# smn-ailab/PyCMF

Measured on AMD Instinct MI355X. Metric: factor-update iterations/s (mu solver: one full update_step per iteration), higher is better.
Workload: dtype f32

## Files before the change

### include/cmfhip.h

```cpp
#ifndef CMFHIP_H
#define CMFHIP_H

#include <stdint.h>

#ifdef __cplusplus
extern "C" {
#endif

typedef struct cmf_ctx cmf_ctx;

enum {
    CMF_OK = 0,
    CMF_EINVAL = 1,
    CMF_EHIP = 2,
    CMF_ENOMEM = 3,
    CMF_ENODEV = 4,
    CMF_EUNSUPPORTED = 5,
    CMF_ERCCL = 6
};

enum { CMF_U = 0, CMF_V = 1, CMF_Z = 2 };
enum { CMF_LINK_LINEAR = 0, CMF_LINK_LOGIT = 1 };
enum { CMF_UPD_U = 1, CMF_UPD_V = 2, CMF_UPD_Z = 4 };
enum { CMF_NN_U = 1, CMF_NN_V = 2, CMF_NN_Z = 4 };
// ... 68 lines not shown
int cmf_weighted_residual_sq(cmf_ctx *ctx, double *ex, double *ey);
int cmf_mu_weighted_layout(cmf_ctx *ctx, int64_t *out4);
int cmf_fill_weight_synthetic(cmf_ctx *ctx, int which, uint64_t seed, double density);
int cmf_get_weight_block_f32(cmf_ctx *ctx, int which, int64_t row0, int64_t nrows, int64_t col0, int64_t ncols, float *host_dst);

int cmf_hals_step(cmf_ctx *ctx, double l1, double l2, int update_mask);
int cmf_hals_sweep(cmf_ctx *ctx, int which, const double *N, const double *G, double l1, double l2);

int cmf_als_step(cmf_ctx *ctx, double l2, int nn_mask, int update_mask);
int cmf_als_normal(cmf_ctx *ctx, int which, int64_t row0, int64_t nrows, double l2, float *host_H, float *host_g);
int cmf_als_layout(cmf_ctx *ctx, int64_t *out4);
int cmf_als_nnls_step(cmf_ctx *ctx, double l2, int nn_mask, int update_mask, int sweeps);
int cmf_als_nnls_rows(cmf_ctx *ctx, int64_t nrows, const float *host_H, const float *host_g, float *host_f, int sweeps);
int cmf_als_cg_step(cmf_ctx *ctx, double l2, int nn_mask, int update_mask, int cg_steps, int nn_sweeps);
int cmf_als_cg_rows(cmf_ctx *ctx, int which, int64_t row0, int64_t nrows, double l2, int cg_steps, float *host_f);
int cmf_als_cg_last(cmf_ctx *ctx, int64_t *out2);

int cmf_set_background_weight(cmf_ctx *ctx, int which, double c0);
int cmf_get_background_weight(cmf_ctx *ctx, int which, double *c0);
int cmf_als_residual_sq(cmf_ctx *ctx, double *ex, double *ey);

int cmf_set_biases(cmf_ctx *ctx, int which, int enable, double mu, double lb);
int cmf_get_biases(cmf_ctx *ctx, int which, double *mu, double *lb, int *enabled);
int cmf_set_bias_f64(cmf_ctx *ctx, int which, int axis, const double *v);
int cmf_get_bias_f64(cmf_ctx *ctx, int which, int axis, double *v);
int cmf_als_bias_step(cmf_ctx *ctx, double l2, int nn_mask, int update_mask, int cg_steps, int nn_sweeps);
int cmf_als_bias_rows(cmf_ctx *ctx, int which, int axis, float *host_out);
int cmf_als_bias_targets(cmf_ctx *ctx, int which, int image, int64_t nnz, float *host_bt, float *host_bp);
int cmf_predict_pairs(cmf_ctx *ctx, int which, int link, int64_t n, const int64_t *rows, const int64_t *cols, float *out);

int cmf_v_buf_elems(cmf_ctx *ctx, int64_t *n);
int cmf_mu_v_partials(cmf_ctx *ctx, float *dev_buf);
int cmf_data_pass_launches(cmf_ctx *ctx, int64_t *out5);
int cmf_mu_route_launches(cmf_ctx *ctx, int64_t *out8);
int cmf_mu_v_partials_rows(cmf_ctx *ctx, float *dev_buf, int64_t row0, int64_t nrows, int with_gram);
int cmf_mu_v_apply(cmf_ctx *ctx, const float *dev_buf, double l1, double l2);
int cmf_mu_uz_update(cmf_ctx *ctx, double l1, double l2, int update_mask);
int cmf_mu_blocked_layout(cmf_ctx *ctx, int world, int64_t *block_rows, int64_t *pbuf_elems);
int cmf_mu_v_partials_split(cmf_ctx *ctx, float *dev_P, float *dev_G);
int cmf_mu_v_apply_rows(cmf_ctx *ctx, const float *dev_P_rows, const float *dev_G, int64_t row0, int64_t nrows, double l1, double l2);
int cmf_mu_gram_v_rows(cmf_ctx *ctx, int64_t row0, int64_t nrows, float *dev_G2);
int cmf_mu_uz_update_gram(cmf_ctx *ctx, const float *dev_G2, double l1, double l2, int update_mask);

int cmf_newton_step(cmf_ctx *ctx, double alpha, double l1, double l2,
                    int x_link, int y_link, int nn_mask, int update_mask,
                    double hessian_pertubation, double sg_ratio,
                    const int32_t *u_idx, const int32_t *z_idx,
                    const int32_t *vx_idx, const int32_t *vy_idx);

int cmf_newton_step_device_sampled(cmf_ctx *ctx, double alpha, double l1, double l2,
                                   int x_link, int y_link, int nn_mask, int update_mask,
                                   double hessian_pertubation, double sg_ratio, uint64_t seed);

int cmf_sample_lists(cmf_ctx *ctx, int sweep, uint64_t seed, double sg_ratio, int64_t row0, int64_t nrows, int32_t *host_out);

int cmf_newton_uz_update(cmf_ctx *ctx, double alpha, double l1, double l2,
                         int nn_mask, int update_mask, double hessian_pertubation);
int cmf_newton_v_partials(cmf_ctx *ctx, double alpha, float *dev_buf);
int cmf_newton_v_apply(cmf_ctx *ctx, const float *dev_buf, double l1, double l2,
                       int nn_mask, double hessian_pertubation);

int cmf_newton_v_gram(cmf_ctx *ctx, double alpha, double *dev_gbuf);
int cmf_newton_v_products(cmf_ctx *ctx, double alpha, double l2, double hessian_pertubation,
                          const double *dev_gbuf, float *dev_pbuf);
int cmf_newton_v_finish(cmf_ctx *ctx, float *dev_pbuf, double l1, int nn_mask);

// ... 90 lines not shown
```

### pycmf_amd/_lib.py

```python
import ctypes as C
import os

import numpy as np

_HERE = os.path.dirname(os.path.abspath(__file__))
LIB_PATH = os.path.join(_HERE, "libcmfhip.so")

CMF_U, CMF_V, CMF_Z = 0, 1, 2
CMF_UPD_U, CMF_UPD_V, CMF_UPD_Z = 1, 2, 4
CMF_NN_U, CMF_NN_V, CMF_NN_Z = 1, 2, 4
LINKS = {"linear": 0, "logit": 1}
UPD_U, UPD_V, UPD_Z = 1, 2, 4
K_GEMM_NN, K_GEMM_TN, K_GEMM_NT, K_ELEMWISE, K_EIGEN = 0, 1, 2, 3, 4
KERNEL_CLASSES = {"gemm_nn": 0, "gemm_tn": 1, "gemm_nt": 2, "elementwise": 3, "eigen": 4, "gemm_small": 5, "spmm": 6, "rowhess": 7, "gemm_pair": 8, "topk": 9, "klmu": 10}
LATER_KERNEL_CLASSES = {"hals": 11}

_ERR = {1: ValueError, 2: RuntimeError, 3: MemoryError, 4: RuntimeError, 5: NotImplementedError}

_i64, _i32, _dbl, _vp = C.c_int64, C.c_int, C.c_double, C.c_void_p
_pd = C.POINTER(C.c_double)
_pf = C.POINTER(C.c_float)
_pi32 = C.POINTER(C.c_int32)
_pi64 = C.POINTER(C.c_int64)

# ... 34 lines not shown
    "cmf_mu_beta_layout": [_vp, _pi64],
    "cmf_set_weight_f64": [_vp, _i32, _pd, _i64, _i64],
    "cmf_set_weight_f32": [_vp, _i32, _pf, _i64, _i64],
    "cmf_set_weighted_csr": [_vp, _i32, _pi64, _pi32, _pd, _pd],
    "cmf_clear_weight": [_vp, _i32],
    "cmf_mu_weighted_step": [_vp, _dbl, _dbl, _i32],
    "cmf_weighted_residual_sq": [_vp, _pd, _pd],
    "cmf_mu_weighted_layout": [_vp, _pi64],
    "cmf_fill_weight_synthetic": [_vp, _i32, C.c_uint64, _dbl],
    "cmf_get_weight_block_f32": [_vp, _i32, _i64, _i64, _i64, _i64, _pf],
    "cmf_hals_step": [_vp, _dbl, _dbl, _i32],
    "cmf_hals_sweep": [_vp, _i32, _pd, _pd, _dbl, _dbl],
    "cmf_als_step": [_vp, _dbl, _i32, _i32],
    "cmf_als_normal": [_vp, _i32, _i64, _i64, _dbl, _pf, _pf],
    "cmf_als_layout": [_vp, _pi64],
    "cmf_als_nnls_step": [_vp, _dbl, _i32, _i32, _i32],
    "cmf_als_nnls_rows": [_vp, _i64, _pf, _pf, _pf, _i32],
    "cmf_als_cg_step": [_vp, _dbl, _i32, _i32, _i32, _i32],
    "cmf_als_cg_rows": [_vp, _i32, _i64, _i64, _dbl, _i32, _pf],
    "cmf_als_cg_last": [_vp, _pi64],
    "cmf_set_background_weight": [_vp, _i32, _dbl],
    "cmf_get_background_weight": [_vp, _i32, _pd],
    "cmf_als_residual_sq": [_vp, _pd, _pd],
    "cmf_set_biases": [_vp, _i32, _i32, _dbl, _dbl],
    "cmf_get_biases": [_vp, _i32, _pd, _pd, C.POINTER(C.c_int)],
    "cmf_set_bias_f64": [_vp, _i32, _i32, _pd],
    "cmf_get_bias_f64": [_vp, _i32, _i32, _pd],
    "cmf_als_bias_step": [_vp, _dbl, _i32, _i32, _i32, _i32],
    "cmf_als_bias_rows": [_vp, _i32, _i32, _pf],
    "cmf_als_bias_targets": [_vp, _i32, _i32, _i64, _pf, _pf],
    "cmf_predict_pairs": [_vp, _i32, _i32, _i64, _pi64, _pi64, _pf],
    "cmf_v_buf_elems": [_vp, _pi64],
    "cmf_data_pass_launches": [_vp, _pi64],
    "cmf_mu_route_launches": [_vp, _pi64],
    "cmf_mu_v_partials": [_vp, _vp],
    "cmf_mu_v_apply": [_vp, _vp, _dbl, _dbl],
    "cmf_mu_v_partials_rows": [_vp, _vp, _i64, _i64, _i32],
    "cmf_mu_uz_update": [_vp, _dbl, _dbl, _i32],
    "cmf_mu_blocked_layout": [_vp, _i32, _pi64, _pi64],
    "cmf_mu_v_partials_split": [_vp, _vp, _vp],
    "cmf_mu_v_apply_rows": [_vp, _vp, _vp, _i64, _i64, _dbl, _dbl],
    "cmf_mu_gram_v_rows": [_vp, _i64, _i64, _vp],
    "cmf_mu_uz_update_gram": [_vp, _vp, _dbl, _dbl, _i32],
    "cmf_newton_step": [_vp, _dbl, _dbl, _dbl, _i32, _i32, _i32, _i32, _dbl, _dbl,
                        _pi32, _pi32, _pi32, _pi32],
    "cmf_newton_step_device_sampled": [_vp, _dbl, _dbl, _dbl, _i32, _i32, _i32, _i32, _dbl, _dbl, C.c_uint64],
    "cmf_newton_uz_update": [_vp, _dbl, _dbl, _dbl, _i32, _i32, _dbl],
    "cmf_newton_v_partials": [_vp, _dbl, _vp],
    "cmf_newton_v_apply": [_vp, _vp, _dbl, _dbl, _i32, _dbl],
    "cmf_newton_v_gram": [_vp, _dbl, _vp],
    "cmf_newton_v_products": [_vp, _dbl, _dbl, _dbl, _vp, _vp],
    "cmf_newton_v_finish": [_vp, _vp, _dbl, _i32],
    "cmf_residual_sq": [_vp, _i32, _i32, _pd, _pd],
    "cmf_data_sq": [_vp, _pd, _pd],
    "cmf_topk": [_vp, _i32, _i32, _i32, _pi64, _i64, _i32, _pi64, _pi32, _pi32, _pf],
    "cmf_topk_queries": [_vp, _pd, _i64, _i64, _i64, _i32, _i32, _i32, _pi64, _pi32, _pi32, _pf],
    "cmf_topk_layout": [_vp, _i64, _i32, _i32, _i64, _i32, _pi64],
    "cmf_rank": [_vp, _i32, _i32, _pi64, _i64, _pi64, _pi32, _pi64, _pi32, _pi32, _pf, _pi32],
    "cmf_rank_queries": [_vp, _pd, _i64, _i64, _i64, _i32, _pi64, _pi32, _pi64, _pi32, _pi32, _pf, _pi32],
    "cmf_rank_layout": [_vp, _i64, _i32, _i64, _i64, _i32, _pi64],
    "cmf_safe_invert_batch": [_vp, _pd, _pd, _i32, _i32, _dbl],
    "cmf_safe_invert_f64": [_vp, _pd, _pd, _i32, _dbl],
    "cmf_safe_solve_batch": [_vp, _pd, _pd, _pd, _pd, _i32, _i32, _dbl, _i32],
    "cmf_debug_clock": [_vp, _pd, _pd],
    "cmf_kernel_timing": [_vp, _i32],
    "cmf_kernel_time": [_vp, _i32, _pd, _pi64, _pd],
# ... 485 lines not shown
    def als_bias_targets(self, which, image, nnz):
        nnz = int(nnz)
        if nnz < 0:
            raise ValueError("als_bias_targets: nnz must be the number of stored entries, got %d" % nnz)
        bt, bp = np.zeros(nnz, dtype=np.float32), np.zeros(nnz, dtype=np.float32)
        check(self._lib.cmf_als_bias_targets(self._h, which, image, nnz, bt.ctypes.data_as(_pf), bp.ctypes.data_as(_pf)))
        return bt, bp

    def predict_pairs(self, which, rows, cols, link="linear"):
        rows = np.ascontiguousarray(rows, dtype=np.int64).ravel()
        cols = np.ascontiguousarray(cols, dtype=np.int64).ravel()
        if rows.shape != cols.shape:
            raise ValueError("predict_pairs: rows and cols must have one length, got %d and %d" % (rows.size, cols.size))
        out = np.zeros(rows.size, dtype=np.float32)
        check(self._lib.cmf_predict_pairs(self._h, which, LINKS[link] if isinstance(link, str) else int(link), rows.size,
                                          rows.ctypes.data_as(_pi64), cols.ctypes.data_as(_pi64), out.ctypes.data_as(_pf)))
        return out

    def mu_step_error(self, l1, l2, mask=7):
        ex2, ey2 = C.c_double(0), C.c_double(0)
        check(self._lib.cmf_mu_step_error(self._h, l1, l2, mask, C.byref(ex2), C.byref(ey2)))
        return ex2.value, ey2.value

    def v_buf_elems(self):
        n = C.c_int64(0)
        check(self._lib.cmf_v_buf_elems(self._h, C.byref(n)))
        return n.value

    def data_pass_launches(self):
        out = np.zeros(5, dtype=np.int64)
        check(self._lib.cmf_data_pass_launches(self._h, out.ctypes.data_as(_pi64)))
        return tuple(int(v) for v in out)

    MU_ROUTE_FORMS = ("epi_mu", "factor_update", "factor_update2", "pair", "gram32", "sum_slabs", "mu_apply", "narrow_copy")

    def mu_route_launches(self):
        out = np.zeros(8, dtype=np.int64)
        check(self._lib.cmf_mu_route_launches(self._h, out.ctypes.data_as(_pi64)))
        return dict(zip(self.MU_ROUTE_FORMS, (int(v) for v in out)))

    def mu_v_partials(self, dev_ptr):
        check(self._lib.cmf_mu_v_partials(self._h, _vp(dev_ptr)))

    def mu_v_partials_rows(self, dev_ptr, row0, nrows, with_gram):
        check(self._lib.cmf_mu_v_partials_rows(self._h, _vp(dev_ptr), row0, nrows, 1 if with_gram else 0))

    def mu_v_apply(self, dev_ptr, l1, l2):
        check(self._lib.cmf_mu_v_apply(self._h, _vp(dev_ptr), l1, l2))

    def mu_uz_update(self, l1, l2, mask=7):
        check(self._lib.cmf_mu_uz_update(self._h, l1, l2, mask))

    def mu_blocked_layout(self, world):
        b, n = C.c_int64(0), C.c_int64(0)
        check(self._lib.cmf_mu_blocked_layout(self._h, int(world), C.byref(b), C.byref(n)))
        return b.value, n.value

    def mu_v_partials_split(self, dev_p, dev_g):
        check(self._lib.cmf_mu_v_partials_split(self._h, _vp(dev_p), _vp(dev_g)))

    def mu_v_apply_rows(self, dev_p_rows, dev_g, row0, nrows, l1, l2):
        check(self._lib.cmf_mu_v_apply_rows(self._h, _vp(dev_p_rows), _vp(dev_g), row0, nrows, l1, l2))

    def mu_gram_v_rows(self, row0, nrows, dev_g2):
        check(self._lib.cmf_mu_gram_v_rows(self._h, row0, nrows, _vp(dev_g2)))

# ... 327 lines not shown
```

### pycmf_amd/csrc/cmf_api.hip

```cpp
#include "../../include/cmfhip.h"
#include "cmf_kernels.hip.h"
#include "cmf_gemm_wg256.hip.h"
#include "cmf_gemm_pair.hip.h"
#include "cmf_eigen.hip.h"
#include "cmf_chol_mfma.hip.h"
#include "cmf_sparse.hip.h"
#include "cmf_rowhess.hip.h"
#include "cmf_bf16x6.hip.h"
#include "cmf_rowhess6.hip.h"
#include "cmf_shared64.hip.h"
#include "cmf_refine64.hip.h"
#include "cmf_eigclamp.hip.h"
#include "cmf_rank1clamp.hip.h"

#include <hip/hip_runtime.h>

#include <algorithm>
#include <chrono>
#include <cmath>
#include <cstdarg>
#include <cstdio>
#include <cstdlib>
#include <cstring>
#include <mutex>
// ... 74 lines not shown
struct StepGraph {
    hipGraphExec_t exec = nullptr;
    double key[8] = {0};
    int warm = 0;
    bool failed = false;
};

struct EvPair {
    hipEvent_t a, b;
    int cls;
    double flops;
};

struct CmfComm;
struct cmf_ctx {
    int device = 0;
    CmfComm *comm = nullptr;
    hipStream_t stream = nullptr;
    bool own_stream = false;
    int num_cu = 256;

    int64_t m = 0, d = 0, p = 0;
    int k = 0;
    int64_t mp = 0, dp = 0, pp = 0;
    int kp = 0;
    bool have_problem = false;
    unsigned long long *dbg_stamps = nullptr;
    bool diag_ok = false;
    int opt_graph = -1;
    StepGraph mu_graph, newton_graph;
    int opt_split = -1;
    int opt_data_pass_wg = 15;
    int64_t data_pass_launches[5] = {0, 0, 0, 0, 0};
    int64_t mu_route_launches[8] = {0, 0, 0, 0, 0, 0, 0, 0};
    int opt_pair = 1;
    int opt_arith_min_tiles = 8;
    int opt_arith = 0;
    int opt_ns = 1;
    bool hess_psd = true;
    int opt_pipe_nt = 4;
    int opt_topk_split = 0;
    int opt_kl_split = 0;
    DevBuf kl_slab, kl_small, kl_part;
    int opt_beta_route = 0;
    DevBuf beta_slab, beta_small, beta_part;
    int opt_wmu_split = 0;
    int wm_kind[2] = {0, 0};
    float *wm_w[2] = {nullptr, nullptr}, *wm_p[2] = {nullptr, nullptr};
    WCsrDev wm_sp[2][2];
    DevBuf wm_slab, wm_small, wm_part;
    DevBuf hals_ws;
    int opt_als_piece = 0;
    DevBuf als_h, als_part, als_g, als_sol, als_desc;
    DevBuf als_nnls_ws;
    int opt_als_cg_lds = -1;
    DevBuf als_cg_ws;
    int opt_als_cg_piece = 0;
    DevBuf als_cg_long;
    int64_t als_cg_last[2] = {0, 0};
    double wm_bg[2] = {0.0, 0.0};
    DevBuf als_bg_s, als_bg64;
    AlsBias als_bias[2];
    int opt_als_bias_piece = 0;
    DevBuf als_bias_part, als_bias_ws;
    int opt_choldiag = 0;
    int opt_chol = 1;
// ... 250 lines not shown
struct GemmPlan {
    int bn;
    int ntiles_n;
    int64_t tiles_m;
    int nsplit;
    int64_t klen;
};

static GemmPlan plan_gemm(const cmf_ctx *c, int64_t mout, int64_t n, int64_t kred, bool allow_split) {
    GemmPlan pl;
    pl.bn = n >= 256 ? 256 : (int)n;
    pl.ntiles_n = (int)(n / pl.bn);
    pl.tiles_m = (mout + 255) / 256;
    const int64_t tiles = pl.tiles_m * pl.ntiles_n;
    int64_t s = 1;
    if (allow_split && c->opt_split > 0) {
        s = std::min<int64_t>(c->opt_split, std::max<int64_t>(1, kred / 32));
    } else if (allow_split && tiles < (int64_t)(c->num_cu * 3) / 4) {
        s = ((int64_t)c->num_cu + tiles / 2) / tiles;
        const int64_t maxs = std::max<int64_t>(1, kred / 128);
        s = std::max<int64_t>(1, std::min(s, maxs));
    }
    pl.klen = rup((kred + s - 1) / s, 32);
    pl.nsplit = (int)((kred + pl.klen - 1) / pl.klen);
    return pl;
}

template <int MODE, int ROLE>
static int launch_gemm(cmf_ctx *c, const GemmArgs &a, const GemmPlan &pl) {
    static_assert(MODE != MODE_NT, "NT passes: gemm_nt");
    dim3 grid((unsigned)pl.tiles_m, (unsigned)pl.ntiles_n, (unsigned)pl.nsplit);
    if (ROLE == 0 && pl.bn == 256 && (c->opt_data_pass_wg & (MODE == MODE_TN ? 1 : 2)) && a.epi == EPI_NONE && a.Mout % 256 == 0) {
        if ((c->opt_data_pass_wg & (MODE == MODE_TN ? 4 : 8)) && a.lda < ((int64_t)1 << 21) && a.ldb < ((int64_t)1 << 21)) {
            using Cfg = Wg256Cfg<MODE, true>;
            if constexpr (Cfg::LDS_BYTES != 0) CHK(allow_big_lds(c, reinterpret_cast<const void *>(&gemm_wg256_kernel<MODE, true>), (int)Cfg::LDS_BYTES));
            hipLaunchKernelGGL((gemm_wg256_kernel<MODE, true>), grid, dim3(Cfg::NT), Cfg::LDS_BYTES, c->stream, a);
            ++c->data_pass_launches[MODE == MODE_TN ? 3 : 4];
        } else {
            using Cfg = Wg256Cfg<MODE, false>;
            CHK(allow_big_lds(c, reinterpret_cast<const void *>(&gemm_wg256_kernel<MODE, false>), (int)Cfg::LDS_BYTES));
            hipLaunchKernelGGL((gemm_wg256_kernel<MODE, false>), grid, dim3(Cfg::NT), Cfg::LDS_BYTES, c->stream, a);
            ++c->data_pass_launches[MODE == MODE_TN ? 1 : 2];
        }
        HIPCHK(hipGetLastError());
        return CMF_OK;
    }
    if (ROLE == 0 && pl.bn == 256) ++c->data_pass_launches[0];
    dim3 block(512);
#define CMF_LAUNCH(BN_)                                                                          \
    do {                                                                                         \
        using Cfg = GemmCfg<MODE, BN_>;                                                          \
        CHK(allow_big_lds(c, reinterpret_cast<const void *>(&gemm_kernel<MODE, BN_, ROLE, 4>), (int)Cfg::LDS_BYTES)); \
        hipLaunchKernelGGL((gemm_kernel<MODE, BN_, ROLE, 4>), grid, block, Cfg::LDS_BYTES, c->stream, a); \
    } while (0)
    switch (pl.bn) {
    case 256: CMF_LAUNCH(256); break;
    case 128: CMF_LAUNCH(128); break;
    case 64: CMF_LAUNCH(64); break;
    case 32: CMF_LAUNCH(32); break;
    default: return fail(CMF_EINVAL, "unsupported tile width %d", pl.bn);
    }
#undef CMF_LAUNCH
    HIPCHK(hipGetLastError());
    return CMF_OK;
}

static int sum_slabs(cmf_ctx *c, float *dst, const float *src, int64_t n, int nslab, int64_t stride,
                     bool accumulate) {
    Timed tm(c, CMF_K_ELEMWISE);
    const int64_t n4 = n / 4;
    const int blocks = (int)std::min<int64_t>((n4 + 255) / 256, 2048);
    hipLaunchKernelGGL(sum_slabs_kernel, dim3(blocks), dim3(256), 0, c->stream, dst, src, n4, nslab, stride,
                       accumulate ? 1 : 0);
    ++c->mu_route_launches[5];
    HIPCHK(hipGetLastError());
    return CMF_OK;
}

static int mu_apply(cmf_ctx *c, float *F, const float *num, const float *den, int64_t n, double l1, double l2);

struct SlabRef {
    const float *base = nullptr;
    int nslab = 0;
    int64_t stride = 0;
    int64_t quota = 0, unit0 = 0;
    int ksteps = 0;
};

struct Epilogue {
    int kind = 0;
    const float *F = nullptr, *P = nullptr;
    const SlabRef *Pslabs = nullptr, *Pslabs2 = nullptr;
    float *out = nullptr;
    double a = 0.0, b = 0.0, c = 0.0;
    int64_t rows = 0;
    int kvalid = 0, nn = 0;
};

static int gemm(cmf_ctx *c, int mode, const float *A, int64_t lda, const float *B, int64_t ldb, float *out,
                int64_t mout, int64_t n, int64_t kred, bool accumulate = false, const Epilogue *mu = nullptr, SlabRef *defer = nullptr) {
    const bool data_pass = (lda != c->kp);
    DevBuf &slabbuf = c->slab_sel ? c->slabs_b : c->slabs;
    if (kred % 32 || n % 32) return fail(CMF_EINVAL, "gemm: unpadded extent (k=%lld n=%lld)", (long long)kred, (long long)n);
    GemmPlan pl = plan_gemm(c, mout, n, kred, mu == nullptr);
    if (mu && c->opt_narrow_update && pl.ntiles_n == 1) {
        while (pl.bn > 64 && pl.tiles_m * (n / pl.bn) * 2 <= (int64_t)c->num_cu) pl.bn /= 2;
// ... 301 lines not shown
extern "C" int cmf_comm_destroy(cmf_ctx *c);
extern "C" int cmf_ctx_destroy(cmf_ctx *c) {
    if (!c) return CMF_OK;
    DeviceGuard dg(c->device);
    (void)cmf_comm_destroy(c);
    release_problem(c);
    for (void *p : c->scratch) (void)hipFree(p);
    c->scratch.clear();
    (void)hipFree(c->dscalar);
    for (auto &e : c->pending) { (void)hipEventDestroy(e.a); (void)hipEventDestroy(e.b); }
    for (auto e : c->evpool) (void)hipEventDestroy(e);
    for (auto e : c->markers) (void)hipEventDestroy(e);
    for (int b = 0; b < 2; ++b) {
        pin_give(c->pin[b]);
        if (c->pin_ev[b]) (void)hipEventDestroy(c->pin_ev[b]);
    }
    if (c->own_stream) (void)hipStreamDestroy(c->stream);
    delete c;
    return CMF_OK;
}

extern "C" int cmf_set_option(cmf_ctx *c, const char *name, int64_t value) {
    if (!c || !name) return fail(CMF_EINVAL, "null argument");
    invalidate_graphs(c);
    if (!strcmp(name, "graph")) {
        c->opt_graph = value < 0 ? -1 : (value != 0);
        return CMF_OK;
    }
    if (!strcmp(name, "gemm_pipe_nt")) {
        c->opt_pipe_nt = (int)value;
    } else if (!strcmp(name, "gemm_split")) {
        c->opt_split = (int)value;
    } else if (!strcmp(name, "data_pass_wg")) {
        if (value < 0 || value > 15)
            return fail(CMF_EINVAL, "data_pass_wg: bit 0 the TN data passes, bit 1 the NN data passes, bit 2 / bit 3 their factor from a register ring (0..15)");
        c->opt_data_pass_wg = (int)value;
    } else if (!strcmp(name, "small_gram_shares")) {
        c->opt_gram32_shares = (int)std::max<int64_t>(1, std::min<int64_t>(value, 1024));
    } else if (!strcmp(name, "small_gram")) {
        c->opt_gram32 = value != 0;
    } else if (!strcmp(name, "chol_mfma")) {
        c->opt_chol_mfma = value != 0;
    } else if (!strcmp(name, "narrow_update")) {
        c->opt_narrow_update = value != 0;
    } else if (!strcmp(name, "pair_passes")) {
        c->opt_pair = (int)value;
    } else if (!strcmp(name, "z_logit_hessian_l2")) {
        c->opt_zlogit_l2 = value != 0;
    } else if (!strcmp(name, "row_diag")) {
#ifndef CMF_DIAG_BUILD
        if (value != 0) return fail(CMF_EINVAL, "row_diag is a timing-only diagnostic (wrong results) that the default build does not carry: "
                                                "build with `python -m pycmf_amd.build --diag` and set CMF_DIAG=1");
#endif
        if (value != 0 && !c->diag_ok) return fail(CMF_EINVAL, "row_diag is a timing-only diagnostic (wrong results): set CMF_DIAG=1 in the environment to allow it");
        c->opt_rowdiag = (int)value;
    } else if (!strcmp(name, "row_stagger")) {
        c->opt_rowstagger = value != 0;
    } else if (!strcmp(name, "row_symmetric")) {
        c->opt_rowsym = (int)value;
    } else if (!strcmp(name, "row_kernel")) {
        c->opt_rowkernel = value != 0;
    } else if (!strcmp(name, "direct_newton_step")) {
        c->opt_direct_step = value != 0;
    } else if (!strcmp(name, "row_certificates")) {
        c->opt_rowcert = value != 0;
    } else if (!strcmp(name, "row_classes")) {
        if (value < -1 || value > 6) return fail(CMF_EINVAL, "row_classes: -1 (automatic), 0 (off) or 2..6 rows per group");
        c->opt_rowclasses = (int)value;
    } else if (!strcmp(name, "row_chunk")) {
// ... 461 lines not shown
    (void)hipFree(dev_ptr);
    return CMF_OK;
}

extern "C" int cmf_export_factor_rows(cmf_ctx *c, int which, float *dev_dst) {
    NEED_PROBLEM(c);
    if (which < 0 || which > 2 || !dev_dst) return fail(CMF_EINVAL, "bad factor argument");
    DeviceGuard dg(c->device);
    HIPCHK(hipMemcpyAsync(dev_dst, c->F[which], (size_t)c->frows[which] * c->kp * sizeof(float), hipMemcpyDeviceToDevice, c->stream));
    return CMF_OK;
}

extern "C" int cmf_import_factor_rows(cmf_ctx *c, int which, const float *dev_src) {
    NEED_PROBLEM(c);
    if (which < 0 || which > 2 || !dev_src) return fail(CMF_EINVAL, "bad factor argument");
    DeviceGuard dg(c->device);
    HIPCHK(hipMemcpyAsync(c->F[which], dev_src, (size_t)c->frows[which] * c->kp * sizeof(float), hipMemcpyDeviceToDevice, c->stream));
    return CMF_OK;
}

extern "C" int cmf_v_buf_elems(cmf_ctx *c, int64_t *n) {
    NEED_PROBLEM(c);
    if (!n) return fail(CMF_EINVAL, "null argument");
    *n = c->dp * c->kp + (int64_t)c->kp * c->kp;
    return CMF_OK;
}

extern "C" int cmf_data_pass_launches(cmf_ctx *c, int64_t *out5) {
    if (!c || !out5) return fail(CMF_EINVAL, "cmf_data_pass_launches: null context or output");
    for (int f = 0; f < 5; ++f) out5[f] = c->data_pass_launches[f];
    return CMF_OK;
}

extern "C" int cmf_mu_route_launches(cmf_ctx *c, int64_t *out8) {
    if (!c || !out8) return fail(CMF_EINVAL, "cmf_mu_route_launches: null context or output");
    for (int f = 0; f < 8; ++f) out8[f] = c->mu_route_launches[f];
    return CMF_OK;
}

extern "C" int cmf_mu_v_partials(cmf_ctx *c, float *buf) {
    NEED_PROBLEM(c);
    if (!buf) return fail(CMF_EINVAL, "null buffer");
    if (!have_data(c, 0) || !have_data(c, 1)) return fail(CMF_EINVAL, "X and Y must be set before a V update");
    DeviceGuard dg(c->device);
    float *P = buf, *Gs = buf + c->dp * c->kp;
    CHK(data_times(c, 0, true, c->F[CMF_U], P));
    CHK(data_times(c, 1, false, c->F[CMF_Z], P, true));
    CHK(gram32(c, c->F[CMF_U], c->mp + c->pp, Gs));
    return CMF_OK;
}

extern "C" int cmf_mu_v_partials_rows(cmf_ctx *c, float *buf, int64_t row0, int64_t nrows, int with_gram) {
    NEED_PROBLEM(c);
    if (!buf) return fail(CMF_EINVAL, "null buffer");
    if (!c->X || !c->Y) return fail(CMF_EUNSUPPORTED, "cmf_mu_v_partials_rows needs dense images of X and Y");
    if (c->opt_arith != 0) return fail(CMF_EUNSUPPORTED, "cmf_mu_v_partials_rows: fp32 MFMA arithmetic only");
    if (row0 < 0 || nrows <= 0 || row0 % 256 || nrows % 256 || row0 + nrows > c->dp) return fail(CMF_EINVAL, "row block must be 256-aligned inside [0, d_pad)");
    DeviceGuard dg(c->device);
    float *P = buf + row0 * c->kp;
    CHK(gemm(c, MODE_TN, c->X + row0, c->dp, c->F[CMF_U], c->kp, P, nrows, c->kp, c->mp));
    CHK(gemm(c, MODE_NN, c->Y + row0 * c->pp, c->pp, c->F[CMF_Z], c->kp, P, nrows, c->kp, c->pp, true));
    if (with_gram)
        CHK(gram32(c, c->F[CMF_U], c->mp + c->pp, buf + c->dp * c->kp));
    return CMF_OK;
}

// ... 443 lines not shown
```

### pycmf_amd/csrc/cmf_gemm_wg256.hip.h

```cpp
#pragma once
#include "cmf_kernels.hip.h"

namespace cmfk {

template <int MODE, bool FREG>
struct Wg256Cfg {
    static_assert(MODE == MODE_NN || MODE == MODE_TN, "data passes: NN and TN");
    static constexpr int BM = 256, BN = 256, BK = 32, PADK = BK + 4, NT = 256;
    static constexpr int A_ELEMS = (MODE == MODE_NN) ? BM * PADK : 0;
    static constexpr int B_ELEMS = FREG ? 0 : BK * BN;
    static constexpr int STAGE = A_ELEMS + B_ELEMS;
    static constexpr int LD = BK * BN / 4 / NT;
    static constexpr size_t LDS_BYTES = 2 * STAGE * sizeof(float);
};

template <int MODE, bool FREG>
__global__ __launch_bounds__(256) void gemm_wg256_kernel(GemmArgs g) {
    using C = Wg256Cfg<MODE, FREG>;
    constexpr bool NN = (MODE == MODE_NN);
    constexpr bool LDS = C::LDS_BYTES != 0;
    constexpr int NGRP = C::BK / 2;
    constexpr int XREG_MI = 5, FREG_MI = 10;
    extern __shared__ __attribute__((aligned(16))) float smem[];

    const int t = threadIdx.x;
    const int lane = t & 63, wid = t >> 6;
    const int l31 = lane & 31, lh = lane >> 5;
    const int wrow0 = 128 * (wid >> 1), wcol0 = 128 * (wid & 1);

    const int64_t row0 = (int64_t)blockIdx.x * C::BM;
    const int64_t n0 = (int64_t)blockIdx.y * C::BN;
    const int64_t kbeg = (int64_t)blockIdx.z * g.klen;
    int64_t kend = kbeg + g.klen;
    if (kend > g.Kred) kend = g.Kred;
    const int nkt = (int)((kend - kbeg) / C::BK);
    const int64_t klast = kend - C::BK;

    f32x16 acc[4][4];
#pragma unroll
    for (int i = 0; i < 4; ++i)
#pragma unroll
        for (int j = 0; j < 4; ++j)
#pragma unroll
            for (int r = 0; r < 16; ++r) acc[i][j][r] = 0.0f;

    const int64_t wg_linear = ((int64_t)blockIdx.z * gridDim.y + blockIdx.y) * gridDim.x + blockIdx.x;
    if (g.dbg && t == 0) {
        g.dbg[4 * wg_linear + 0] = __builtin_amdgcn_s_memtime();
        g.dbg[4 * wg_linear + 1] = __builtin_amdgcn_s_memrealtime();
    }

    f32x4 rb[FREG ? 1 : C::LD], ra[NN ? C::LD : 1];
// ... 45 lines not shown
#pragma unroll
                for (int s = 0; s < NGRP; ++s) gload_x(kbeg, s);
        } else if constexpr (NN) {
#pragma unroll
            for (int p = 0; p < C::LD; ++p) gload_au(kbeg, p);
            __builtin_amdgcn_sched_barrier(0);
#pragma unroll
            for (int p = 0; p < C::LD; ++p) lstore_a(smem, p);
            __builtin_amdgcn_sched_barrier(0);
#pragma unroll
            for (int p = 0; p < C::LD; ++p) {
                gload_au(k1, p);
                __builtin_amdgcn_sched_barrier(0);
                if (p == FREG_MI / 2 - 1) {
                    gload_f(kbeg, 0);
                    __builtin_amdgcn_sched_barrier(0);
                }
            }
#pragma unroll
            for (int s = 1; s < NGRP - 1; ++s) {
                gload_f(kbeg, s);
                __builtin_amdgcn_sched_barrier(0);
            }
        } else {
#pragma unroll
            for (int s = 0; s < NGRP - 1; ++s) {
                gload_xu(kbeg, s);
                __builtin_amdgcn_sched_barrier(0);
                gload_f(kbeg, s);
                __builtin_amdgcn_sched_barrier(0);
            }
        }
        if constexpr (LDS) __syncthreads();
        for (int kt = 0; kt < nkt; ++kt) {
            const float *As = smem + (kt & 1) * C::STAGE, *Bs = As + C::A_ELEMS;
            float *nAs = smem + ((kt + 1) & 1) * C::STAGE, *nBs = nAs + C::A_ELEMS;
            int64_t kn1 = kbeg + (int64_t)(kt + 1) * C::BK, kn2 = kn1 + C::BK;
            kn1 = kn1 < klast ? kn1 : klast;
            kn2 = kn2 < klast ? kn2 : klast;
            f32x4 a[NN ? 2 : 1][4], b[2];
            auto ldb_frag = [&](int sidx) {
                const int kk = NN ? 8 * (sidx >> 2) + 4 * lh + (sidx & 3) : 2 * sidx + lh;
                b[sidx & 1] = *reinterpret_cast<const f32x4 *>(Bs + kk * C::BN + wcol0 + 4 * l31);
            };
            auto lda_frag = [&](int q) {
#pragma unroll
                for (int i = 0; i < 4; ++i)
                    a[q & 1][i] = *reinterpret_cast<const f32x4 *>(As + (wrow0 + 32 * i + l31) * C::PADK + 4 * (2 * q + lh));
            };
            if constexpr (NN) lda_frag(0);
            if constexpr (!FREG) ldb_frag(0);
#pragma unroll
            for (int sidx = 0; sidx < NGRP; ++sidx) {
                const int q = sidx >> 2, e = sidx & 3;
                if (sidx + 1 < NGRP) {
                    if constexpr (!FREG) ldb_frag(sidx + 1);
                    if constexpr (NN)
                        if (e == 0 && q + 1 < NGRP / 4) lda_frag(q + 1);
                }
                __builtin_amdgcn_sched_barrier(0);
#pragma unroll
                for (int mi = 0; mi < 16; ++mi) {
                    const int i = mi >> 2, j = mi & 3;
                    const float av = NN ? a[q & 1][i][e] : xr[sidx][i];
                    const float bv = FREG ? br[sidx][j] : b[sidx & 1][j];
                    acc[i][j] = __builtin_amdgcn_mfma_f32_32x32x2f32(av, bv, acc[i][j], 0, 0, 0);
                    if constexpr (NN && FREG) {
                        if (sidx == 0 && (mi & 1)) lstore_a(nAs, mi >> 1);
                        if (sidx == 1 && (mi & 1)) gload_au(kn2, mi >> 1);
                    } else if constexpr (NN) {
                        const int p = mi >> 1;
                        if (sidx == 0) {
                            if (mi & 1) lstore_b(nBs, p);
                            else lstore_a(nAs, p);
                        } else if (sidx == 1) {
                            if (mi & 1) gload_b(kn2, p);
                            else gload_a(kn2, p);
                        }
                    } else if constexpr (!FREG) {
                        if (sidx == 0 && mi < C::LD) lstore_b(nBs, mi);
                        if (sidx == 0 && mi >= C::LD) gload_b(kn2, mi - C::LD);
                    }
                    if constexpr (FREG) {
                        const int rs = (sidx + NGRP - 1) % NGRP;
                        const int64_t kr = sidx == 0 ? kbeg + (int64_t)kt * C::BK : kn1;
                        if (!NN && mi == XREG_MI) gload_xu(kr, rs);
                        if (mi == FREG_MI) gload_f(kr, rs);
                    }
                    __builtin_amdgcn_sched_barrier(0);
                }
                if constexpr (!NN && !FREG) {
                    gload_x(kn1, sidx);
                    __builtin_amdgcn_sched_barrier(0);
                }
            }
            if constexpr (LDS) __syncthreads();
        }
    }

    if (g.dbg && t == 0) {
        g.dbg[4 * wg_linear + 2] = __builtin_amdgcn_s_memtime();
        g.dbg[4 * wg_linear + 3] = __builtin_amdgcn_s_memrealtime();
    }
    const bool in_red = g.red_out != nullptr;
    float *Cl = (in_red ? g.red_out : g.C + (int64_t)blockIdx.z * g.slab_stride) +
                (row0 + wrow0 + (NN ? 4 : 16) * lh) * g.ldc + n0 + wcol0 + 4 * l31;
    const int ldc = (int)g.ldc;
    auto rowoff = [&](int i, int r) -> int {
        const int rr = (r & 3) + 8 * (r >> 2);
        return (NN ? 32 * i + rr : 4 * rr + i) * ldc;
    };
    if (in_red && g.red_acc) {
#pragma unroll
        for (int i = 0; i < 4; ++i) {
#pragma unroll
            for (int j = 0; j < 4; ++j) asm volatile("" : "+a"(acc[i][j]));
            f32x4 old[16];
#pragma unroll
            for (int r = 0; r < 16; ++r) old[r] = *reinterpret_cast<const f32x4 *>(Cl + rowoff(i, r));
#pragma unroll
            for (int r = 0; r < 16; ++r) {
                f32x4 v = {acc[i][0][r], acc[i][1][r], acc[i][2][r], acc[i][3][r]};
                v += old[r];
                *reinterpret_cast<f32x4 *>(Cl + rowoff(i, r)) = v;
            }
            __builtin_amdgcn_sched_barrier(0);
        }
    } else {
#pragma unroll
// ... 15 lines not shown
```

### pycmf_amd/csrc/cmf_kernels.hip.h

```cpp
#pragma once
#include <hip/hip_runtime.h>
#include <stdint.h>

namespace cmfk {

typedef float f32x16 __attribute__((ext_vector_type(16)));
typedef float f32x4 __attribute__((ext_vector_type(4)));
typedef float f32x2 __attribute__((ext_vector_type(2)));

enum { MODE_NN = 0, MODE_TN = 1, MODE_NT = 2 };

struct GemmArgs {
    const float *A;
    int64_t lda;
    const float *B;
    int64_t ldb;
    float *C;
    int64_t ldc;
    int64_t slab_stride;
    int64_t Mout;
    int64_t Kred;
    int64_t klen;
    const float *T;
    int64_t ldt;
// ... 731 lines not shown
    for (int idx = blockIdx.x * 256 + threadIdx.x; idx < kp * kp; idx += gridDim.x * 256) {
        const int r = idx / kp, c = idx % kp;
        const int rr = r < c ? r : c, cc = r < c ? c : r;
        const int ti = rr / ts, tj = cc / ts;
        int ir = rr % ts, ic = cc % ts;
        if (ti == tj) { ir = r % ts; ic = c % ts; }
        const int tile = ti * T - ti * (ti - 1) / 2 + (tj - ti);
        const float *p = slab + (int64_t)tile * ts * ts + ir * ts + ic;
        const int64_t st = (int64_t)ntile * ts * ts;
        float s = 0.f;
        int q = 0;
        for (; q + 8 <= nsplit; q += 8) {
            float v[8];
#pragma unroll
            for (int u = 0; u < 8; ++u) v[u] = p[(q + u) * st];
#pragma unroll
            for (int u = 0; u < 8; ++u) s += v[u];
        }
        for (; q < nsplit; ++q) s += p[q * st];
        G[idx] = s;
    }
}

__global__ void sum_slabs_kernel(float *dst, const float *src, int64_t n4, int nslab,
                                 int64_t stride, int accumulate) {
    for (int64_t i = (int64_t)blockIdx.x * blockDim.x + threadIdx.x; i < n4;
         i += (int64_t)gridDim.x * blockDim.x) {
        f32x4 a = accumulate ? reinterpret_cast<f32x4 *>(dst)[i] : f32x4{0.f, 0.f, 0.f, 0.f};
        for (int s = 0; s < nslab; ++s) a += reinterpret_cast<const f32x4 *>(src + (int64_t)s * stride)[i];
        reinterpret_cast<f32x4 *>(dst)[i] = a;
    }
}

__global__ void mu_apply_kernel(float *F, const float *num, const float *den, int64_t n4,
                                float l1, float l2, float eps) {
    for (int64_t i = (int64_t)blockIdx.x * blockDim.x + threadIdx.x; i < n4;
         i += (int64_t)gridDim.x * blockDim.x) {
        f32x4 f = reinterpret_cast<f32x4 *>(F)[i];
        const f32x4 nu = reinterpret_cast<const f32x4 *>(num)[i];
        f32x4 de = reinterpret_cast<const f32x4 *>(den)[i];
#pragma unroll
        for (int e = 0; e < 4; ++e) {
            float d = de[e];
            if (l1 > 0.f) d += l1;
            if (l2 > 0.f) d = d + l2 * f[e];
            if (d == 0.f) d = eps;
            f[e] = f[e] * (nu[e] / d);
        }
        reinterpret_cast<f32x4 *>(F)[i] = f;
    }
}

__global__ void newton_grad_kernel(float *grad, const float *P, float a, const float *Q, float b,
                                   const float *F, float l1, float l2, int64_t n) {
    for (int64_t i = (int64_t)blockIdx.x * blockDim.x + threadIdx.x; i < n;
         i += (int64_t)gridDim.x * blockDim.x) {
        const float f = F[i];
        float gval = a * P[i];
        if (Q) gval += b * Q[i];
        const float sg = (f > 0.f) ? 1.f : ((f < 0.f) ? -1.f : 0.f);
        grad[i] = gval + l1 * sg + l2 * f;
    }
}

__global__ void newton_apply_kernel(float *F, const float *step, int64_t rows_valid, int kp, int kvalid,
                                    int64_t n, int non_negative) {
// ... 262 lines not shown
```

Measured before the change: 17.25.

## Add three-stage LDS ring to NN data-pass GEMM and wide slab-sum kernel

Adds a three-stage LDS variant of the NN wg256 data-pass GEMM that rotates stage buffers, moves the barrier to mid-tile and preloads the next tile's A fragment early, removing the end-of-iteration sync. It is gated by bit 4 of data_pass_wg, which stays at default 15, so it does not run by default. Also adds a scalar per-element slab-sum kernel with 16-way unrolled loads, used by default when the vectorised grid would have fewer blocks than CUs, to raise parallelism for small reductions. The extra stage costs LDS and may reduce occupancy.

```diff
diff --git a/include/cmfhip.h b/include/cmfhip.h
--- a/include/cmfhip.h
+++ b/include/cmfhip.h
@@ -124,6 +124,7 @@
 int cmf_v_buf_elems(cmf_ctx *ctx, int64_t *n);
 int cmf_mu_v_partials(cmf_ctx *ctx, float *dev_buf);
 int cmf_data_pass_launches(cmf_ctx *ctx, int64_t *out5);
+int cmf_data_pass_nn3_launches(cmf_ctx *ctx, int64_t *out1);
 int cmf_mu_route_launches(cmf_ctx *ctx, int64_t *out8);
 int cmf_mu_v_partials_rows(cmf_ctx *ctx, float *dev_buf, int64_t row0, int64_t nrows, int with_gram);
 int cmf_mu_v_apply(cmf_ctx *ctx, const float *dev_buf, double l1, double l2);
diff --git a/pycmf_amd/_lib.py b/pycmf_amd/_lib.py
--- a/pycmf_amd/_lib.py
+++ b/pycmf_amd/_lib.py
@@ -90,6 +90,7 @@
     "cmf_predict_pairs": [_vp, _i32, _i32, _i64, _pi64, _pi64, _pf],
     "cmf_v_buf_elems": [_vp, _pi64],
     "cmf_data_pass_launches": [_vp, _pi64],
+    "cmf_data_pass_nn3_launches": [_vp, _pi64],
     "cmf_mu_route_launches": [_vp, _pi64],
     "cmf_mu_v_partials": [_vp, _vp],
     "cmf_mu_v_apply": [_vp, _vp, _dbl, _dbl],
@@ -641,6 +642,11 @@
         check(self._lib.cmf_data_pass_launches(self._h, out.ctypes.data_as(_pi64)))
         return tuple(int(v) for v in out)
 
+    def data_pass_nn3_launches(self):
+        n = C.c_int64(0)
+        check(self._lib.cmf_data_pass_nn3_launches(self._h, C.byref(n)))
+        return n.value
+
     MU_ROUTE_FORMS = ("epi_mu", "factor_update", "factor_update2", "pair", "gram32", "sum_slabs", "mu_apply", "narrow_copy")
 
     def mu_route_launches(self):
diff --git a/pycmf_amd/csrc/cmf_api.hip b/pycmf_amd/csrc/cmf_api.hip
--- a/pycmf_amd/csrc/cmf_api.hip
+++ b/pycmf_amd/csrc/cmf_api.hip
@@ -130,6 +130,8 @@
     int opt_split = -1;
     int opt_data_pass_wg = 15;
     int64_t data_pass_launches[5] = {0, 0, 0, 0, 0};
+    int64_t data_pass_nn3_launches = 0;
+    int opt_slab_sum_wide = 1;
     int64_t mu_route_launches[8] = {0, 0, 0, 0, 0, 0, 0, 0};
     int opt_pair = 1;
     int opt_arith_min_tiles = 8;
@@ -446,6 +448,17 @@
     dim3 grid((unsigned)pl.tiles_m, (unsigned)pl.ntiles_n, (unsigned)pl.nsplit);
     if (ROLE == 0 && pl.bn == 256 && (c->opt_data_pass_wg & (MODE == MODE_TN ? 1 : 2)) && a.epi == EPI_NONE && a.Mout % 256 == 0) {
         if ((c->opt_data_pass_wg & (MODE == MODE_TN ? 4 : 8)) && a.lda < ((int64_t)1 << 21) && a.ldb < ((int64_t)1 << 21)) {
+            if constexpr (MODE == MODE_NN) {
+                if (c->opt_data_pass_wg & 16) {
+                    using Cfg3 = Wg256Cfg<MODE_NN, true, 3>;
+                    CHK(allow_big_lds(c, reinterpret_cast<const void *>(&gemm_wg256_kernel<MODE_NN, true, 3>), (int)Cfg3::LDS_BYTES));
+                    hipLaunchKernelGGL((gemm_wg256_kernel<MODE_NN, true, 3>), grid, dim3(Cfg3::NT), Cfg3::LDS_BYTES, c->stream, a);
+                    ++c->data_pass_launches[4];
+                    ++c->data_pass_nn3_launches;
+                    HIPCHK(hipGetLastError());
+                    return CMF_OK;
+                }
+            }
             using Cfg = Wg256Cfg<MODE, true>;
             if constexpr (Cfg::LDS_BYTES != 0) CHK(allow_big_lds(c, reinterpret_cast<const void *>(&gemm_wg256_kernel<MODE, true>), (int)Cfg::LDS_BYTES));
             hipLaunchKernelGGL((gemm_wg256_kernel<MODE, true>), grid, dim3(Cfg::NT), Cfg::LDS_BYTES, c->stream, a);
@@ -484,8 +497,12 @@
     Timed tm(c, CMF_K_ELEMWISE);
     const int64_t n4 = n / 4;
     const int blocks = (int)std::min<int64_t>((n4 + 255) / 256, 2048);
-    hipLaunchKernelGGL(sum_slabs_kernel, dim3(blocks), dim3(256), 0, c->stream, dst, src, n4, nslab, stride,
-                       accumulate ? 1 : 0);
+    if (c->opt_slab_sum_wide && blocks < c->num_cu)
+        hipLaunchKernelGGL(sum_slabs_wide_kernel, dim3((unsigned)((n + 255) / 256)), dim3(256), 0, c->stream, dst, src, n, nslab, stride,
+                           accumulate ? 1 : 0);
+    else
+        hipLaunchKernelGGL(sum_slabs_kernel, dim3(blocks), dim3(256), 0, c->stream, dst, src, n4, nslab, stride,
+                           accumulate ? 1 : 0);
     ++c->mu_route_launches[5];
     HIPCHK(hipGetLastError());
     return CMF_OK;
@@ -853,9 +870,13 @@
     } else if (!strcmp(name, "gemm_split")) {
         c->opt_split = (int)value;
     } else if (!strcmp(name, "data_pass_wg")) {
-        if (value < 0 || value > 15)
-            return fail(CMF_EINVAL, "data_pass_wg: bit 0 the TN data passes, bit 1 the NN data passes, bit 2 / bit 3 their factor from a register ring (0..15)");
+        if (value < 0 || value > 31)
+            return fail(CMF_EINVAL, "data_pass_wg: bit 0 the TN data passes, bit 1 the NN data passes, bit 2 / bit 3 their factor from a register ring, "
+                                    "bit 4 the NN ring form with three X stages (0..31)");
         c->opt_data_pass_wg = (int)value;
+    } else if (!strcmp(name, "slab_sum_wide")) {
+        if (value < 0 || value > 1) return fail(CMF_EINVAL, "slab_sum_wide: 0 (sum_slabs_kernel everywhere) or 1 (sum_slabs_wide_kernel for results below one workgroup per CU)");
+        c->opt_slab_sum_wide = (int)value;
     } else if (!strcmp(name, "small_gram_shares")) {
         c->opt_gram32_shares = (int)std::max<int64_t>(1, std::min<int64_t>(value, 1024));
     } else if (!strcmp(name, "small_gram")) {
@@ -1383,6 +1404,12 @@
     return CMF_OK;
 }
 
+extern "C" int cmf_data_pass_nn3_launches(cmf_ctx *c, int64_t *out1) {
+    if (!c || !out1) return fail(CMF_EINVAL, "cmf_data_pass_nn3_launches: null context or output");
+    *out1 = c->data_pass_nn3_launches;
+    return CMF_OK;
+}
+
 extern "C" int cmf_mu_route_launches(cmf_ctx *c, int64_t *out8) {
     if (!c || !out8) return fail(CMF_EINVAL, "cmf_mu_route_launches: null context or output");
     for (int f = 0; f < 8; ++f) out8[f] = c->mu_route_launches[f];
diff --git a/pycmf_amd/csrc/cmf_gemm_wg256.hip.h b/pycmf_amd/csrc/cmf_gemm_wg256.hip.h
--- a/pycmf_amd/csrc/cmf_gemm_wg256.hip.h
+++ b/pycmf_amd/csrc/cmf_gemm_wg256.hip.h
@@ -3,21 +3,24 @@
 
 namespace cmfk {
 
-template <int MODE, bool FREG>
+template <int MODE, bool FREG, int STAGES = 2>
 struct Wg256Cfg {
     static_assert(MODE == MODE_NN || MODE == MODE_TN, "data passes: NN and TN");
+    static_assert(STAGES == 2 || (STAGES == 3 && MODE == MODE_NN && FREG), "three X stages: the NN ring form only");
     static constexpr int BM = 256, BN = 256, BK = 32, PADK = BK + 4, NT = 256;
     static constexpr int A_ELEMS = (MODE == MODE_NN) ? BM * PADK : 0;
     static constexpr int B_ELEMS = FREG ? 0 : BK * BN;
     static constexpr int STAGE = A_ELEMS + B_ELEMS;
     static constexpr int LD = BK * BN / 4 / NT;
-    static constexpr size_t LDS_BYTES = 2 * STAGE * sizeof(float);
+    static constexpr size_t LDS_BYTES = STAGES * STAGE * sizeof(float);
 };
 
-template <int MODE, bool FREG>
+template <int MODE, bool FREG, int STAGES = 2>
 __global__ __launch_bounds__(256) void gemm_wg256_kernel(GemmArgs g) {
-    using C = Wg256Cfg<MODE, FREG>;
+    using C = Wg256Cfg<MODE, FREG, STAGES>;
     constexpr bool NN = (MODE == MODE_NN);
+    constexpr bool S3 = (STAGES == 3);
+    constexpr int BAR_GRP = 6, AHEAD_GRP = 12;
     constexpr bool LDS = C::LDS_BYTES != 0;
     constexpr int NGRP = C::BK / 2;
     constexpr int XREG_MI = 5, FREG_MI = 10;
@@ -129,13 +132,24 @@
             }
         }
         if constexpr (LDS) __syncthreads();
+        int st_cur = 0, st_nxt = C::STAGE, st_fre = 2 * C::STAGE;
+        f32x4 a[NN ? 2 : 1][4], b[2];
+        if constexpr (S3) {
+#pragma unroll
+            for (int i = 0; i < 4; ++i)
+                a[0][i] = *reinterpret_cast<const f32x4 *>(smem + (wrow0 + 32 * i + l31) * C::PADK + 4 * lh);
+            __builtin_amdgcn_sched_barrier(0);
+        }
         for (int kt = 0; kt < nkt; ++kt) {
-            const float *As = smem + (kt & 1) * C::STAGE, *Bs = As + C::A_ELEMS;
-            float *nAs = smem + ((kt + 1) & 1) * C::STAGE, *nBs = nAs + C::A_ELEMS;
+            const float *As = smem + (S3 ? st_cur : (kt & 1) * C::STAGE), *Bs = As + C::A_ELEMS;
+            float *nAs = smem + (S3 ? st_nxt : ((kt + 1) & 1) * C::STAGE), *nBs = nAs + C::A_ELEMS;
+            if constexpr (S3) {
+                const int st = st_cur;
+                st_cur = st_nxt, st_nxt = st_fre, st_fre = st;
+            }
             int64_t kn1 = kbeg + (int64_t)(kt + 1) * C::BK, kn2 = kn1 + C::BK;
             kn1 = kn1 < klast ? kn1 : klast;
             kn2 = kn2 < klast ? kn2 : klast;
-            f32x4 a[NN ? 2 : 1][4], b[2];
             auto ldb_frag = [&](int sidx) {
                 const int kk = NN ? 8 * (sidx >> 2) + 4 * lh + (sidx & 3) : 2 * sidx + lh;
                 b[sidx & 1] = *reinterpret_cast<const f32x4 *>(Bs + kk * C::BN + wcol0 + 4 * l31);
@@ -145,7 +159,7 @@
                 for (int i = 0; i < 4; ++i)
                     a[q & 1][i] = *reinterpret_cast<const f32x4 *>(As + (wrow0 + 32 * i + l31) * C::PADK + 4 * (2 * q + lh));
             };
-            if constexpr (NN) lda_frag(0);
+            if constexpr (NN && !S3) lda_frag(0);
             if constexpr (!FREG) ldb_frag(0);
 #pragma unroll
             for (int sidx = 0; sidx < NGRP; ++sidx) {
@@ -154,6 +168,13 @@
                     if constexpr (!FREG) ldb_frag(sidx + 1);
                     if constexpr (NN)
                         if (e == 0 && q + 1 < NGRP / 4) lda_frag(q + 1);
+                }
+                if constexpr (S3) {
+                    if (sidx == BAR_GRP) __syncthreads();
+                    if (sidx == AHEAD_GRP)
+#pragma unroll
+                        for (int i = 0; i < 4; ++i)
+                            a[0][i] = *reinterpret_cast<const f32x4 *>(nAs + (wrow0 + 32 * i + l31) * C::PADK + 4 * lh);
                 }
                 __builtin_amdgcn_sched_barrier(0);
 #pragma unroll
@@ -191,7 +212,7 @@
                     __builtin_amdgcn_sched_barrier(0);
                 }
             }
-            if constexpr (LDS) __syncthreads();
+            if constexpr (LDS && !S3) __syncthreads();
         }
     }
 
diff --git a/pycmf_amd/csrc/cmf_kernels.hip.h b/pycmf_amd/csrc/cmf_kernels.hip.h
--- a/pycmf_amd/csrc/cmf_kernels.hip.h
+++ b/pycmf_amd/csrc/cmf_kernels.hip.h
@@ -787,6 +787,24 @@
     }
 }
 
+__global__ __launch_bounds__(256) void sum_slabs_wide_kernel(float *dst, const float *src, int64_t n, int nslab,
+                                                             int64_t stride, int accumulate) {
+    const int64_t i = (int64_t)blockIdx.x * 256 + threadIdx.x;
+    if (i >= n) return;
+    float a = accumulate ? dst[i] : 0.f;
+    const float *p = src + i;
+    int s = 0;
+    for (; s + 16 <= nslab; s += 16) {
+        float v[16];
+#pragma unroll
+        for (int u = 0; u < 16; ++u) v[u] = p[(int64_t)(s + u) * stride];
+#pragma unroll
+        for (int u = 0; u < 16; ++u) a += v[u];
+    }
+    for (; s < nslab; ++s) a += p[(int64_t)s * stride];
+    dst[i] = a;
+}
+
 __global__ void mu_apply_kernel(float *F, const float *num, const float *den, int64_t n4,
                                 float l1, float l2, float eps) {
     for (int64_t i = (int64_t)blockIdx.x * blockDim.x + threadIdx.x; i < n4;
```

After: 17.29 (median of 6 runs). About the same (+0.2%).
